# quan-dao/practical-collab-perception

Measured on AMD Instinct MI355X. Metric: frames/sec (60k-pt cloud, 6 agents), higher is better.
Workload: dtype f32

## Files before the change

include/pcp_hip.h:

```cpp
#ifndef PCP_HIP_H
#define PCP_HIP_H

#include <stddef.h>
#include <stdint.h>

#ifdef __cplusplus
extern "C" {
#endif

#define PCP_ABI_VERSION 1

enum {
  PCP_OK = 0,
  PCP_ERR_ARG = 1,
  PCP_ERR_WORKSPACE = 2,
  PCP_ERR_LAUNCH = 3,
  PCP_ERR_UNSUPPORTED = 4
};

int pcp_abi_version(void);
const char *pcp_status_string(int status);

enum {
  PCP_OPT_PFN_CROWD = 0,
  PCP_OPT_PFN_CROWD_BLOCKS = 1,
  PCP_OPT_PFN_WPS = 2,
  PCP_OPT_WINO4C_NW = 3,
  PCP_OPT_MP_TH16_MIN = 4,
  PCP_OPT_MP_DIAG = 5,
  PCP_OPT_VOX_AGGREGATE = 6,
  PCP_OPT_CONV_S2_FORM = 7,
  PCP_OPT_GTS_PASTE_FORM = 8,
  PCP_OPT_COUNT = 9
};
int pcp_set_option(int32_t option, int64_t value);
int64_t pcp_get_option(int32_t option);

typedef struct {
  float min_x, min_y, min_z;
  float voxel_x, voxel_y, voxel_z;
  int32_t nx, ny;
  int32_t batch_size;
} pcp_grid_t;

#define PCP_VOX_COUNTERS 4

size_t pcp_voxelize_workspace_bytes(const pcp_grid_t *grid, int64_t max_points);

int pcp_voxelize(const float *points, int64_t n, int32_t row_stride, const pcp_grid_t *grid,
                 void *workspace, size_t workspace_bytes,
                 int32_t *voxel_coords, int64_t *unq_inv, int32_t *unq_cnt, int32_t *counters, void *stream);
int pcp_voxelize_cells_ready(const float *points, int64_t n, int32_t row_stride, const pcp_grid_t *grid,
                             void *workspace, size_t workspace_bytes,
                             int32_t *voxel_coords, int32_t *unq_cnt, int32_t *counters, void *stream);

int pcp_voxelize_sort_pillar_rows(const pcp_grid_t *grid, void *workspace, int64_t n, void *stream);
int pcp_voxelize_row_order(const pcp_grid_t *grid, const void *workspace, int64_t n, int32_t *order, int32_t *cursor_scratch,
                           void *stream);

int pcp_pfn_scatter(const float *points, int64_t n, int32_t row_stride, int32_t num_raw, const pcp_grid_t *grid,
                    const void *workspace, const float *w0, const float *b0, const float *w1, const float *b1,
                    float *pillar_features, float *canvas, void *stream);

#define PCP_ROWS_CELLS_READY 1
#define PCP_ROWS_BUCKET_ORDER 2
size_t pcp_pillarise_rows_workspace_bytes(const pcp_grid_t *grid, int64_t max_points, int32_t num_raw);
int pcp_pillarise_rows(const float *points, int64_t n, int32_t row_stride, int32_t num_raw, const pcp_grid_t *grid,
                       void *workspace, size_t workspace_bytes, int32_t *voxel_coords, int64_t *unq_inv, int32_t *unq_cnt,
                       int32_t *counters, int32_t flags, void *stream);
int pcp_pfn_rows(const pcp_grid_t *grid, const void *workspace, int64_t n, int32_t num_raw, const float *w0, const float *b0,
                 const float *w1, const float *b1, float *pillar_features, float *canvas, void *stream);
int pcp_pillar_index_export(const pcp_grid_t *grid, const void *workspace, int64_t n, int32_t num_raw, int32_t *voxel_coords,
                            int32_t *row_rank, int32_t *slot_rank, int32_t *slot_canvas_row, int32_t *counters, void *stream);

#define PCP_PFN_ABSOLUTE_XYZ 1u
#define PCP_PFN_WITH_DISTANCE 2u
int pcp_pfn_features(const float *points, int64_t n, int32_t row_stride, int32_t num_raw, uint32_t flags, const pcp_grid_t *grid,
                     const void *vox_workspace, int32_t fw, float *fbuf, int32_t *slot_pillar, void *stream);
int pcp_pfn_cat_pillar_max(const float *y, int32_t ld_y, const float *pillar_max, int32_t ld_max, const int32_t *slot_pillar, int64_t rows,
                           int32_t c, float *out, int32_t ld_out, void *stream);

int pcp_canvas_clear(const pcp_grid_t *grid, const void *workspace, int64_t n, float *canvas, void *stream);
int pcp_fill_zero(void *ptr, size_t bytes, void *stream);

typedef struct {
  int32_t batch, in_h, in_w;
  int32_t cin, cout;
  int32_t cout_pad;
  int32_t stride;
  int32_t ld_in, ld_out;
  int32_t relu;
} pcp_conv3x3_t;

int pcp_conv3x3(const pcp_conv3x3_t *desc, const float *in, const float *w_packed, const float *bias, float *out,
                void *stream);

int pcp_sparse_conv3x3_s2(const float *pillar_features, const pcp_grid_t *grid, const void *vox_workspace, int64_t n,
                          const float *w_packed, const float *bias, int32_t cout, int32_t relu, float *out, int32_t ld_out,
                          void *stream);

int pcp_conv3x3_winograd(const pcp_conv3x3_t *desc, const float *in, const float *u_packed, const float *bias, float *out,
                         void *stream);

int pcp_conv3x3_winograd_ws_supported(const pcp_conv3x3_t *desc);
int pcp_conv3x3_winograd_ws(const pcp_conv3x3_t *desc, const float *in, const float *u_packed, const float *bias, float *out,
                            void *stream);
int pcp_conv3x3_winograd_ws_plan(const pcp_conv3x3_t *desc, int32_t *variant, double *executed_flops);

int pcp_conv3x3_winograd4f(const pcp_conv3x3_t *desc, const float *in, const float *u_packed, const float *bias, float *out,
                           void *stream);
int pcp_conv3x3_winograd4f_plan(const pcp_conv3x3_t *desc, double *executed_flops);

int pcp_conv3x3_winograd4h(const pcp_conv3x3_t *desc, const float *in, const float *u_packed, const float *bias, float *out,
                           void *stream);
int pcp_conv3x3_winograd4h_plan(const pcp_conv3x3_t *desc, double *executed_flops);

int pcp_conv3x3_winograd4c(const pcp_conv3x3_t *desc, const float *in, const float *u_packed, const float *bias, float *out,
                           void *stream);
int pcp_conv3x3_winograd4c_plan(const pcp_conv3x3_t *desc, double *executed_flops);

int pcp_conv3x3_winograd_plan(const pcp_conv3x3_t *desc, int32_t *variant, double *executed_flops);

int pcp_conv3x3_winograd4_workspace_bytes(const pcp_conv3x3_t *desc, size_t *bytes);
int pcp_conv3x3_winograd4(const pcp_conv3x3_t *desc, const float *in, const float *u_packed, const float *bias, float *out,
                          void *workspace, void *stream);
int pcp_conv3x3_winograd4_timed(const pcp_conv3x3_t *desc, const float *in, const float *u_packed, const float *bias, float *out,
                                void *workspace, void *stream, float *stage_ms_host, double *gemm_flops_host);

int pcp_conv3x3_bf16x3(const pcp_conv3x3_t *desc, const float *in, const void *w_packed, const float *bias, float *out, void *stream);
int pcp_conv3x3_bf16(const pcp_conv3x3_t *desc, const float *in, const void *w_packed, const float *bias, float *out, void *stream);

int pcp_conv3x3_grouped_small(const float *in, int32_t batch, int32_t h, int32_t w, int32_t ld_in, int32_t groups,
                              int32_t cin_per_group, const int32_t *group_out_offsets_host, const float *weights, const float *bias, float *out,
                              int32_t ld_out, void *stream);

enum {
  PCP_PW_PLAIN = 0,
  PCP_PW_SPACE2DEPTH = 1,
  PCP_PW_DEPTH2SPACE = 2
};

typedef struct {
  int32_t mode;
  int64_t rows;
  int32_t batch, in_h, in_w;
  int32_t cin, cout, cout_pad;
  int32_t ld_in, ld_out;
  int32_t relu;
  const float *in2;
  int32_t ld_in2, k_split;
  const float *residual;
  int32_t ld_res;
} pcp_pointwise_t;

int pcp_pointwise(const pcp_pointwise_t *desc, const float *in, const float *w_packed, const float *bias, float *out,
                  void *stream);

typedef struct {
  int32_t batch, h, w, ld;
  int32_t num_class;
  int32_t ch_center, ch_z, ch_dim, ch_rot, ch_hm;
  int32_t k;
  float stride;
  float voxel_x, voxel_y, min_x, min_y;
  float limit[6];
  int32_t use_score_thresh;
  float score_thresh;
  int32_t activated;
} pcp_decode_t;

size_t pcp_decode_workspace_bytes(const pcp_decode_t *desc);
int pcp_centerhead_decode(const pcp_decode_t *desc, const float *head, void *workspace, size_t workspace_bytes,
                          float *boxes, float *scores, int32_t *labels, int32_t *cell, int32_t *count, void *stream);

#define PCP_DET_MAX_HEADS 8
typedef struct {
  const float *boxes;
  const float *scores;
  const int32_t *labels;
  const int32_t *keep;
  const int32_t *keep_count;
  const int32_t *class_map;
  int32_t k, keep_max;
} pcp_det_head_t;
int pcp_gather_detections(const pcp_det_head_t *heads, int32_t n_heads, int32_t batch, int32_t out_max, float *out_boxes,
                          float *out_scores, int64_t *out_labels, int32_t *out_count, void *stream);
// ... 129 lines not shown
```

practical-collab-perception_amd/csrc/abi.hip:

```cpp
#include "pcp_common.h"

extern "C" int pcp_abi_version(void) { return PCP_ABI_VERSION; }

extern "C" const char *pcp_status_string(int status) {
  switch (status) {
    case PCP_OK: return "ok";
    case PCP_ERR_ARG: return "bad argument";
    case PCP_ERR_WORKSPACE: return "workspace too small";
    case PCP_ERR_LAUNCH: return "kernel launch failed";
    case PCP_ERR_UNSUPPORTED: return "unsupported shape for this build";
    default: return "unknown status";
  }
}

#include <atomic>

namespace {
std::atomic<long long> g_option[PCP_OPT_COUNT] = {{-1}, {-1}, {-1}, {-1}, {-1}, {-1}, {-1}, {-1}, {-1}};
static_assert(PCP_OPT_COUNT == 9, "one initialiser per option");
constexpr int MAX_DEVICES = 64;
std::atomic<int> g_cus[MAX_DEVICES];
}

extern "C" int pcp_set_option(int32_t option, int64_t value) {
  if (option < 0 || option >= PCP_OPT_COUNT) return PCP_ERR_ARG;
  g_option[option].store(value < 0 ? -1 : (long long)value, std::memory_order_relaxed);
  return PCP_OK;
}

extern "C" int64_t pcp_get_option(int32_t option) {
  if (option < 0 || option >= PCP_OPT_COUNT) return -1;
  return g_option[option].load(std::memory_order_relaxed);
}

long long pcp_option(int option, long long builtin) {
  const long long v = g_option[option].load(std::memory_order_relaxed);
  return v < 0 ? builtin : v;
}

int pcp_current_device_cus() {
  int dev = 0;
  if (hipGetDevice(&dev) != hipSuccess || dev < 0 || dev >= MAX_DEVICES) return 256;
  int v = g_cus[dev].load(std::memory_order_relaxed);
  if (v > 0) return v;
  if (hipDeviceGetAttribute(&v, hipDeviceAttributeMultiprocessorCount, dev) != hipSuccess || v <= 0) v = 256;
  g_cus[dev].store(v, std::memory_order_relaxed);
  return v;
}
```

practical-collab-perception_amd/csrc/wino4c.hip:

```cpp
#include "wino4_common.h"
#include <type_traits>

namespace {

constexpr int H4_LDS_FLOATS = H4_MAIN_FLOATS;
constexpr int H4_VRING = 2;

template <int NW>
__global__ __launch_bounds__(NW * 64, NW == 4 ? 2 : 1) void k_wino4c(H4Params p) {
  constexpr int THREADS = NW * 64;
  constexpr int RAW_PER = (H4_RAW_ITEMS + THREADS - 1) / THREADS;
  constexpr int WBN = NW * 16;
  constexpr int URING = NW == 4 ? H4_URING : 2;
  __shared__ __attribute__((aligned(16))) float lds[H4_LDS_FLOATS];
  float *rawb = lds;
  float *vb = lds + 2 * H4_RAW_FLOATS;

  const int tid = threadIdx.x;
  const int lane = tid & 63;
  const int wave = __builtin_amdgcn_readfirstlane(tid >> 6);
  const int h = lane >> 5;

  const int lid = xcd_remap(blockIdx.x, gridDim.x);
  const int nt = lid / p.n_spatial;
  int sp = lid % p.n_spatial;
  const int tile_x = sp % p.tiles_x;
  sp /= p.tiles_x;
  const int tile_y = sp % p.tiles_y;
  const int b = sp / p.tiles_y;
  const int oy0 = tile_y * 16, ox0 = tile_x * 16;
  const int n0 = nt * WBN;

  const __amdgpu_buffer_rsrc_t in_rsrc = __builtin_amdgcn_make_buffer_rsrc(const_cast<float *>(p.in), 0, p.in_bytes, 0x00020000);
  unsigned roff[RAW_PER];
  int rdst[RAW_PER];
#pragma unroll
  for (int i = 0; i < RAW_PER; i++) {
    int idx = tid + i * THREADS;
    if (idx >= H4_RAW_ITEMS) idx -= H4_RAW_ITEMS;
    const int q = idx & 1, pix = idx >> 1;
    const int py = pix / H4_RAW_W, px = pix % H4_RAW_W;
    const int iy = oy0 - 1 + py, ix = ox0 - 1 + px;
    rdst[i] = (4 * q) * H4_PLANE + py * H4_RP + px;
    roff[i] = 0x80000000u;
    if (iy >= 0 && iy < p.h && ix >= 0 && ix < p.w) roff[i] = (unsigned)((((long long)(b * p.h + iy) * p.w + ix) * p.ld_in + q * 4) * 4);
  }
  f32x4 rreg[RAW_PER];
  auto raw_load = [&](int slice) {
    const int soff = slice * (H4_CK * 4);
#pragma unroll
    for (int i = 0; i < RAW_PER; i++)
      rreg[i] = __builtin_bit_cast(f32x4, __builtin_amdgcn_raw_buffer_load_b128(in_rsrc, (int)roff[i], soff, 0));
  };
  auto raw_store = [&](int buf) {
    float *dst = rawb + buf * H4_RAW_FLOATS;
#pragma unroll
    for (int i = 0; i < RAW_PER; i++) {
      const f32x4 v = rreg[i];
      dst[rdst[i]] = v.x;
      dst[rdst[i] + H4_PLANE] = v.y;
      dst[rdst[i] + 2 * H4_PLANE] = v.z;
      dst[rdst[i] + 3 * H4_PLANE] = v.w;
    }
  };

  const int t_li = lane & 31;
  const bool tf = NW == 4 || wave < 4;
  const int t_tile = t_li & 15, t_ch = 2 * (wave & 3) + (t_li >> 4);
  const int t_src = t_ch * H4_PLANE + (4 * (t_tile >> 2) + 3 * h) * H4_RP + 4 * (t_tile & 3);
  const int t_dst = t_ch * 16 + t_tile + (3 * h) * H4_VP;
  const H4Transform transform{rawb, vb, t_src, t_dst};

  const __amdgpu_buffer_rsrc_t u_rsrc = __builtin_amdgcn_make_buffer_rsrc(const_cast<float *>(p.u), 0, p.u_bytes, 0x00020000);
  const int u_lane = lane * 16;
  const int u_slice = (p.cout_pad / 16) * (18 * 64 * 4 * 4);
  const int u_base = (nt * NW + wave) * (18 * 64 * 4 * 4);
  const int n_slices = p.cin / H4_CK;
  const int last = n_slices - 1;
  f32x4 uq[18];
  auto u_load = [&](int slice, int q) {
    const int so = u_base + min(slice, last) * u_slice + q * (64 * 4 * 4);
    uq[q] = __builtin_bit_cast(f32x4, __builtin_amdgcn_raw_buffer_load_b128(u_rsrc, u_lane, so, 0));
  };

  f32x4 acc[36];
#pragma unroll
  for (int i = 0; i < 36; i++) acc[i] = f32x4{0.f, 0.f, 0.f, 0.f};

  const int v_off = lane;
  float vq[H4_VRING][4][2];
  f32x4 lo[3];
  float2 hi[3];

  auto step_blocks = [&](int s, auto last_tag) {
    constexpr bool LAST = decltype(last_tag)::value;
    const int cur = s & 1, nxt = cur ^ 1;
    const float *vsrc = vb + cur * H4_V_FLOATS + v_off;
    float *tdst = vb + nxt * H4_V_FLOATS + t_dst;
    float *rdstb = rawb + cur * H4_RAW_FLOATS;
    auto mm = [&](int pi) {
      const f32x4 ua = uq[2 * pi], ub = uq[2 * pi + 1];
      float (&v)[4][2] = vq[pi % H4_VRING];
      acc[4 * pi + 0] = __builtin_amdgcn_mfma_f32_16x16x4f32(ua.x, v[0][0], acc[4 * pi + 0], 0, 0, 0);
      acc[4 * pi + 1] = __builtin_amdgcn_mfma_f32_16x16x4f32(ua.z, v[1][0], acc[4 * pi + 1], 0, 0, 0);
      acc[4 * pi + 2] = __builtin_amdgcn_mfma_f32_16x16x4f32(ub.x, v[2][0], acc[4 * pi + 2], 0, 0, 0);
      acc[4 * pi + 3] = __builtin_amdgcn_mfma_f32_16x16x4f32(ub.z, v[3][0], acc[4 * pi + 3], 0, 0, 0);
      acc[4 * pi + 0] = __builtin_amdgcn_mfma_f32_16x16x4f32(ua.y, v[0][1], acc[4 * pi + 0], 0, 0, 0);
      acc[4 * pi + 1] = __builtin_amdgcn_mfma_f32_16x16x4f32(ua.w, v[1][1], acc[4 * pi + 1], 0, 0, 0);
      acc[4 * pi + 2] = __builtin_amdgcn_mfma_f32_16x16x4f32(ub.y, v[2][1], acc[4 * pi + 2], 0, 0, 0);
      acc[4 * pi + 3] = __builtin_amdgcn_mfma_f32_16x16x4f32(ub.w, v[3][1], acc[4 * pi + 3], 0, 0, 0);
      if (pi + H4_VRING < 9) {
#pragma unroll
        for (int j = 0; j < 4; j++) {
          v[j][0] = vsrc[(4 * (pi + H4_VRING) + j) * H4_VP];
          v[j][1] = vsrc[(4 * (pi + H4_VRING) + j) * H4_VP + 64];
        }
      }
#pragma unroll
      for (int e = 0; e < 2; e++) {
        const int q = 2 * (pi + URING) + e;
        if (q < 18) u_load(s, q);
        else if (!LAST) u_load(s + 1, q - 18);
      }
    };
    auto rstore = [&](int i) {
      const f32x4 v = rreg[i];
      rdstb[rdst[i]] = v.x;
      rdstb[rdst[i] + H4_PLANE] = v.y;
      rdstb[rdst[i] + 2 * H4_PLANE] = v.z;
      rdstb[rdst[i] + 3 * H4_PLANE] = v.w;
    };
    const auto fence = [] { __builtin_amdgcn_sched_barrier(0); };
    fence();
    float wr[3][6];
    float top[3][3], bot[3][3];
    auto other = [&](int blk) {
      if (blk == 0) rstore(0);
      if (blk == 1) rstore(1);
      if (blk == 2 && RAW_PER > 2) rstore(RAW_PER > 2 ? 2 : 0);
      if (blk == 3) raw_load(min(s + 3, last));
      if (!tf) return;
      if (blk == 1) bt6(lo[0].x, lo[0].y, lo[0].z, lo[0].w, hi[0].x, hi[0].y, wr[0]);
      if (blk == 2) bt6(lo[1].x, lo[1].y, lo[1].z, lo[1].w, hi[1].x, hi[1].y, wr[1]);
      if (blk == 3) bt6(lo[2].x, lo[2].y, lo[2].z, lo[2].w, hi[2].x, hi[2].y, wr[2]);
      if (blk == 4) {
#pragma unroll
        for (int rr = 0; rr < 3; rr++)
#pragma unroll
          for (int c = 0; c < 3; c++) {
            const auto sw = __builtin_amdgcn_permlane32_swap(__float_as_uint(wr[rr][c]), __float_as_uint(wr[rr][3 + c]), false, false);
            top[rr][c] = __uint_as_float(sw[0]);
            bot[rr][c] = __uint_as_float(sw[1]);
          }
      }
      if (blk >= 5 && blk <= 7) {
        const int c = blk - 5;
        float o[6];
        bt6(top[0][c], top[1][c], top[2][c], bot[0][c], bot[1][c], bot[2][c], o);
#pragma unroll
        for (int i = 0; i < 6; i++) tdst[(i * 6 + c) * H4_VP] = o[i];
      }
    };
#pragma unroll
    for (int blk = 0; blk < 8; blk++) {
      mm(blk);
      fence();
      if (!LAST) {
        other(blk);
        fence();
      }
    }
    if (!LAST) {
      __syncthreads();
      const float *vn = vb + nxt * H4_V_FLOATS + v_off;
      const float *tn = rawb + cur * H4_RAW_FLOATS + t_src;
#pragma unroll
      for (int i = 0; i < H4_VRING; i++)
        if (i != 8 % H4_VRING) {
#pragma unroll
          for (int j = 0; j < 4; j++) {
            vq[i][j][0] = vn[(4 * i + j) * H4_VP];
            vq[i][j][1] = vn[(4 * i + j) * H4_VP + 64];
          }
        }
      if (tf) {
#pragma unroll
        for (int rr = 0; rr < 3; rr++) {
          lo[rr] = *reinterpret_cast<const f32x4 *>(tn + rr * H4_RP);
          hi[rr] = *reinterpret_cast<const float2 *>(tn + rr * H4_RP + 4);
        }
      }
      fence();
      mm(8);
      fence();
#pragma unroll
      for (int j = 0; j < 4; j++) {
        vq[8 % H4_VRING][j][0] = vn[(4 * (8 % H4_VRING) + j) * H4_VP];
        vq[8 % H4_VRING][j][1] = vn[(4 * (8 % H4_VRING) + j) * H4_VP + 64];
      }
      fence();
    } else {
      mm(8);
    }
  };

  {
    f32x4 r0[RAW_PER];
    raw_load(0);
#pragma unroll
    for (int i = 0; i < RAW_PER; i++) r0[i] = rreg[i];
    raw_load(min(1, last));
#pragma unroll
    for (int q = 0; q < 2 * URING; q++) u_load(0, q);
    float *dst = rawb;
#pragma unroll
    for (int i = 0; i < RAW_PER; i++) {
      const f32x4 v = r0[i];
      dst[rdst[i]] = v.x;
      dst[rdst[i] + H4_PLANE] = v.y;
      dst[rdst[i] + 2 * H4_PLANE] = v.z;
      dst[rdst[i] + 3 * H4_PLANE] = v.w;
    }
    if (n_slices > 1) raw_store(1);
    raw_load(min(2, last));
  }
  __syncthreads();
  if (tf) transform(0, 0);
  __syncthreads();
#pragma unroll
  for (int i = 0; i < H4_VRING; i++)
#pragma unroll
    for (int j = 0; j < 4; j++) {
      vq[i][j][0] = vb[v_off + (4 * i + j) * H4_VP];
      vq[i][j][1] = vb[v_off + (4 * i + j) * H4_VP + 64];
    }
  if (tf) {
#pragma unroll
    for (int rr = 0; rr < 3; rr++) {
      lo[rr] = *reinterpret_cast<const f32x4 *>(rawb + H4_RAW_FLOATS + t_src + rr * H4_RP);
      hi[rr] = *reinterpret_cast<const float2 *>(rawb + H4_RAW_FLOATS + t_src + rr * H4_RP + 4);
    }
  }

  for (int s = 0; s < last; s++) step_blocks(s, std::false_type{});
  step_blocks(last, std::true_type{});

  {
    const int e_tile = lane & 15, e_kq = lane >> 4;
    const int n = n0 + 16 * wave + 4 * e_kq;
    if (n < p.cout) {
      const f32x4 bias = *reinterpret_cast<const f32x4 *>(p.bias + n);
      const int py = oy0 + (e_tile >> 2) * 4, px = ox0 + (e_tile & 3) * 4;
      f32x4 t[4][6];
#pragma unroll
      for (int j = 0; j < 6; j++) {
        f32x4 y[4];
        at6v(acc[j], acc[6 + j], acc[12 + j], acc[18 + j], acc[24 + j], acc[30 + j], y);
#pragma unroll
        for (int r = 0; r < 4; r++) t[r][j] = y[r];
      }
#pragma unroll
      for (int r = 0; r < 4; r++) {
        f32x4 y[4];
        at6v(t[r][0], t[r][1], t[r][2], t[r][3], t[r][4], t[r][5], y);
        if (py + r < p.h) {
          float *o = p.out + ((long long)(b * p.h + py + r) * p.w + px) * p.ld_out + n;
#pragma unroll
          for (int c2 = 0; c2 < 4; c2++)
            if (px + c2 < p.w) {
              f32x4 v = y[c2] + bias;
              if (p.relu) {
                v.x = fmaxf(v.x, 0.f);
                v.y = fmaxf(v.y, 0.f);
                v.z = fmaxf(v.z, 0.f);
                v.w = fmaxf(v.w, 0.f);
              }
              __builtin_nontemporal_store(v, reinterpret_cast<f32x4 *>(o + (long long)c2 * p.ld_out));
            }
        }
      }
    }
  }
}

}

extern "C" int pcp_conv3x3_winograd4c(const pcp_conv3x3_t *d, const float *in, const float *u_packed, const float *bias, float *out,
                                      void *stream_) {
  if (!d || !in || !u_packed || !bias || !out) return PCP_ERR_ARG;
  H4Params p;
  int rc = h4_geom(d, &p);
  if (rc != PCP_OK) return rc;
  if ((((uintptr_t)in) & 15) || (((uintptr_t)u_packed) & 15) || (((uintptr_t)out) & 15) || (((uintptr_t)bias) & 15)) return PCP_ERR_ARG;
  p.in = in; p.u = u_packed; p.bias = bias; p.out = out;
  const bool wide = pcp_option(PCP_OPT_WINO4C_NW, 4) == 8 && d->cout_pad % 128 == 0;
  const long long blocks = (long long)p.n_spatial * (d->cout_pad / (wide ? 128 : 64));
  if (blocks <= 0 || blocks > 0x7fffffffLL) return PCP_ERR_ARG;
  if (wide) hipLaunchKernelGGL(k_wino4c<8>, dim3((unsigned)blocks), dim3(512), 0, (hipStream_t)stream_, p);
  else hipLaunchKernelGGL(k_wino4c<4>, dim3((unsigned)blocks), dim3(256), 0, (hipStream_t)stream_, p);
  PCP_CHECK_LAUNCH();
  return PCP_OK;
}

extern "C" int pcp_conv3x3_winograd4c_plan(const pcp_conv3x3_t *d, double *executed_flops) {
  H4Params p;
  int rc = h4_geom(d, &p);
  if (rc != PCP_OK) return rc;
  if (executed_flops) *executed_flops = (double)p.n_spatial * (d->cout_pad / H4_WBN) * 2.0 * 36.0 * 16.0 * d->cin * H4_WBN;
  return PCP_OK;
}
```

practical-collab-perception_amd/pcp_amd/lib.py:

```python
import ctypes
import os

_HERE = os.path.dirname(os.path.abspath(__file__))
LIB_PATH = os.environ.get('PCP_HIP_LIB') or os.path.abspath(os.path.join(_HERE, '..', 'lib', 'libpcp_hip.so'))

c_f = ctypes.c_float
c_i32 = ctypes.c_int32
c_i64 = ctypes.c_int64
c_sz = ctypes.c_size_t
vp = ctypes.c_void_p


class Grid(ctypes.Structure):
    _fields_ = [('min_x', c_f), ('min_y', c_f), ('min_z', c_f), ('voxel_x', c_f), ('voxel_y', c_f), ('voxel_z', c_f),
                ('nx', c_i32), ('ny', c_i32), ('batch_size', c_i32)]


class PackJob(ctypes.Structure):
    _fields_ = [('w', ctypes.c_void_p), ('cout', ctypes.c_int32), ('cin', ctypes.c_int32), ('transpose', ctypes.c_int32),
                ('direct_cout_pad', ctypes.c_int32), ('direct', ctypes.c_void_p), ('winograd', ctypes.c_void_p),
                ('winograd_cout_pad', ctypes.c_int32), ('f4_cout_pad', ctypes.c_int32), ('u4f', ctypes.c_void_p), ('u4h', ctypes.c_void_p),
                ('block_start', ctypes.c_int32), ('reserved', ctypes.c_int32)]


# ... 213 lines not shown
                                             ctypes.POINTER(ctypes.c_uint8), vp, c_i64, vp, c_sz, vp, ctypes.POINTER(Grid), vp, c_sz, vp]),
    'pcp_select_transform_compact_dev': (c_i32, [vp, c_i64, c_i32, c_i32, c_i32, ctypes.POINTER(c_f), c_i32, vp, vp, vp, c_i64, vp, c_sz, vp,
                                                 ctypes.POINTER(Grid), vp, c_sz, vp]),
    'pcp_warp_nearest_batch_dev': (c_i32, [vp, vp, vp, c_i32, c_i32, c_i32, c_i32, c_i32, c_i32, c_i32, vp]),
    'pcp_voxelize_cells_ready': (c_i32, [vp, c_i64, c_i32, ctypes.POINTER(Grid), vp, c_sz, vp, vp, vp, vp]),
    'pcp_gather_detections': (c_i32, [ctypes.POINTER(DetHead), c_i32, c_i32, c_i32, vp, vp, vp, vp, vp]),
    'pcp_nms_workspace_bytes': (c_sz, [c_i32, c_i32]),
    'pcp_nms_rotated': (c_i32, [vp, vp, c_i32, c_i32, vp, c_f, c_i32, c_i32, vp, c_sz, vp, vp, vp]),
    'pcp_nms_normal': (c_i32, [vp, vp, c_i32, c_i32, vp, c_f, c_i32, c_i32, vp, c_sz, vp, vp, vp]),
    'pcp_boxes_bev_pairwise': (c_i32, [vp, c_i32, vp, c_i32, c_i32, vp, vp]),
    'pcp_warp_nearest': (c_i32, [vp, vp, c_i32, c_i32, c_i32, c_i32, c_i32, ctypes.POINTER(c_f), c_i32, vp]),
    'pcp_warp_nearest_batch': (c_i32, [vp, vp, ctypes.POINTER(c_f), c_i32, c_i32, c_i32, c_i32, c_i32, c_i32, c_i32, vp]),
    'pcp_softmax_fuse': (c_i32, [ctypes.POINTER(vp), c_i32, vp, c_i32, c_i64, c_i32, c_i32, c_i32, vp, vp]),
    'pcp_disco_weight_fuse': (c_i32, [ctypes.POINTER(vp), c_i32, c_i32, c_i32, c_i64, vp, vp, vp, vp, vp, vp, vp, c_i32, vp, c_i32, vp]),
    'pcp_disco_weight_fuse_live': (c_i32, [ctypes.POINTER(vp), c_i32, c_i32, c_i32, c_i64, vp, vp, vp, vp, vp, vp, vp, c_i32, ctypes.POINTER(c_i32), vp, vp]),
    'pcp_bev_sample_bilinear': (c_i32, [vp, c_i32, c_i32, c_i32, c_i32, c_i32, vp, c_i64, c_i32, c_f, c_f, c_f, c_f, vp, vp,
                                        c_i32, vp]),
    'pcp_hunter_point_head': (c_i32, [vp, c_i32, c_i32, c_i32, c_i32, c_i32, vp, c_i64, c_i32, c_f, c_f, c_f, c_f, vp, vp, vp, vp, vp,
                                      vp, c_i32, c_i32, vp, c_i32, vp, vp]),
    'pcp_hunter_point_head_ex': (c_i32, [vp, c_i32, c_i32, c_i32, c_i32, c_i32, vp, c_i64, c_i32, c_f, c_f, c_f, c_f, vp, vp, vp, vp, vp,
                                         vp, c_i32, c_i32, vp, c_i32, vp, vp, vp, c_i32, c_f, vp, vp]),
    'pcp_voxelize_row_order': (c_i32, [ctypes.POINTER(Grid), vp, c_i64, vp, vp, vp]),
    'pcp_voxelize_sort_pillar_rows': (c_i32, [ctypes.POINTER(Grid), vp, c_i64, vp]),
    'pcp_hunter_apply_flow': (c_i32, [vp, c_i64, c_i32, vp, c_i32, c_f, vp, vp]),
    'pcp_select_transform_points': (c_i32, [vp, c_i64, c_i32, c_i32, c_f, c_i32, ctypes.POINTER(c_f), ctypes.POINTER(ctypes.c_uint8),
                                            vp, c_i32, vp]),
    'pcp_bev_scatter_mean_workspace_bytes': (c_sz, [c_i32, c_i32, c_i32, c_i64]),
    'pcp_bev_scatter_mean': (c_i32, [vp, c_i64, c_i32, vp, c_i32, c_i32, c_i32, c_i32, c_i32, c_f, c_f, c_f, c_f, vp, c_sz,
                                     vp, c_i32, vp]),
    'pcp_anchor_decode': (c_i32, [ctypes.POINTER(Anchor), vp, vp, vp, vp, vp, vp, vp]),
    'pcp_topk_boxes': (c_i32, [vp, vp, vp, c_i32, c_i64, c_i32, vp, vp, vp, vp, vp, vp]),
    'pcp_points_in_boxes': (c_i32, [vp, c_i32, c_i32, c_i32, vp, c_i32, c_i32, vp, vp]),
    'pcp_hunter_foreground_workspace_bytes': (c_sz, [c_i64]),
    'pcp_hunter_foreground_rows': (c_i32, [vp, c_i64, c_i32, vp, c_i32, c_f, vp, c_sz, vp, vp, vp, vp]),
    'pcp_modar_ingest_batched_workspace_bytes': (c_sz, [c_i32, c_i64]),
    'pcp_modar_ingest_batched': (c_i32, [vp, vp, vp, vp, c_i32, c_i32, vp, c_i32, vp, vp, c_i64, vp, vp, vp, vp, c_sz, vp, vp]),
    'pcp_modar_ingest': (c_i32, [vp, c_i32, vp, c_i32, c_i32, ctypes.POINTER(ctypes.c_double), c_f, vp, vp]),
}

SYMBOLS.update({
    'pcp_bn_workspace_bytes': (c_sz, [c_i32]),
    'pcp_bn_train_stats': (c_i32, [vp, c_i64, c_i32, c_i32, vp, vp, c_f, c_f, vp, vp, vp, vp, vp, vp, vp, vp]),
    'pcp_scale_shift_act': (c_i32, [vp, c_i64, c_i32, c_i32, vp, vp, c_i32, vp, c_i32, vp]),
    'pcp_bn_act_backward': (c_i32, [vp, c_i32, vp, c_i32, c_i64, c_i32, vp, vp, vp, vp, c_i32, vp, vp, vp, c_i32, vp, c_i32, vp]),
    'pcp_colsum': (c_i32, [vp, c_i64, c_i32, c_i32, vp, vp, c_i32, vp]),
    'pcp_bn_train_sums': (c_i32, [vp, c_i64, c_i32, c_i32, vp, vp, vp]),
    'pcp_bn_train_stats_from_sums': (c_i32, [vp, c_i64, c_i32, vp, vp, c_f, c_f, vp, vp, vp, vp, vp, vp, vp]),
    'pcp_bn_bwd_sums': (c_i32, [vp, c_i32, vp, c_i32, c_i64, c_i32, vp, vp, vp, vp, c_i32, vp, vp, vp]),
    'pcp_bn_bwd_apply_from_sums': (c_i32, [vp, c_i32, vp, c_i32, c_i64, c_i32, vp, vp, vp, vp, c_i32, vp, vp, c_i64, vp, vp, vp, c_i32, vp, c_i32, vp]),
    'pcp_accumulate': (c_i32, [vp, c_i32, vp, c_i32, c_i64, c_i32, c_f, vp]),
    'pcp_dilate2x': (c_i32, [vp, c_i32, c_i32, c_i32, c_i32, c_i32, vp, c_i32, vp]),
    'pcp_conv3x3_wgrad_workspace_bytes': (c_sz, [ctypes.POINTER(Conv3x3)]),
    'pcp_conv3x3_wgrad': (c_i32, [ctypes.POINTER(Conv3x3), vp, vp, vp, c_sz, vp, c_i32, vp]),
    'pcp_pointwise_wgrad_workspace_bytes': (c_sz, [c_i64, c_i32, c_i32]),
    'pcp_pointwise_wgrad': (c_i32, [ctypes.POINTER(RowMap), ctypes.POINTER(RowMap), c_i64, vp, c_sz, vp, c_i32, c_i32, vp]),
    'pcp_centerhead_targets': (c_i32, [ctypes.POINTER(Target), vp, c_i32, vp, vp, vp, vp, vp]),
    'pcp_loss_workspace_bytes': (c_sz, []),
    'pcp_centerhead_loss': (c_i32, [ctypes.POINTER(HeadLoss), vp, vp, vp, vp, vp, c_f, vp, vp, vp, vp]),
    'pcp_centerhead_targets_ext': (c_i32, [ctypes.POINTER(Target), ctypes.POINTER(TargetHead), c_i32, vp, c_i32, c_i32, c_i32, vp]),
    'pcp_centerhead_loss_ext_workspace_bytes': (c_sz, [c_i32]),
    'pcp_centerhead_loss_ext': (c_i32, [ctypes.POINTER(HeadLossExt), ctypes.POINTER(HeadLossHead), c_i32, c_f, vp, c_sz, vp, vp, vp]),
    'pcp_anchor_assign_workspace_bytes': (c_sz, [ctypes.POINTER(AnchorAssign), c_i32]),
    'pcp_anchor_assign_targets': (c_i32, [ctypes.POINTER(AnchorAssign), vp, vp, c_i32, vp, c_sz, vp, vp, vp, vp]),
    'pcp_anchor_loss_workspace_bytes': (c_sz, [c_i32]),
    'pcp_anchor_loss': (c_i32, [ctypes.POINTER(AnchorLoss), vp, vp, vp, vp, c_f, vp, c_sz, vp, vp, vp]),
    'pcp_hunter_meta_workspace_bytes': (c_sz, [ctypes.POINTER(HunterMeta), c_i64]),
    'pcp_hunter_meta': (c_i32, [ctypes.POINTER(HunterMeta), vp, c_i64, c_i32, vp, c_sz, vp, vp, vp, vp, vp, vp, vp, vp, vp]),
    'pcp_segment_max': (c_i32, [vp, c_i32, vp, c_i64, vp, c_i64, c_i32, vp, c_i32, vp, vp]),
    'pcp_segment_max_backward': (c_i32, [vp, c_i32, vp, c_i64, c_i32, vp, vp, c_i32, vp]),
    'pcp_rows_scatter_add': (c_i32, [vp, c_i32, vp, c_i64, c_i32, vp, c_i32, vp]),
    'pcp_hunter_local_centroids': (c_i32, [vp, c_i32, vp, vp, c_i32, c_i32, vp, c_sz, vp, vp, c_i32, vp]),
    'pcp_hunter_object_cat': (c_i32, [vp, vp, vp, vp, vp, c_i32, c_i32, vp, c_i32, vp]),
    'pcp_hunter_object_cat_backward': (c_i32, [vp, c_i32, vp, vp, c_i32, c_i32, c_i32, vp, vp, vp]),
    'pcp_hunter_loss_workspace_bytes': (c_sz, [c_i64, c_i32, c_i32, c_i32]),
    'pcp_hunter_losses': (c_i32, [ctypes.POINTER(HunterLoss), vp, c_sz, vp]),
    'pcp_softmax_fuse2_backward': (c_i32, [vp, c_i32, vp, c_i32, vp, c_i32, c_i64, c_i32, vp, c_i32, vp, c_i32, vp]),
    'pcp_bev_scatter_mean_backward': (c_i32, [vp, c_i32, c_i32, c_i32, c_i64, vp, c_i32, c_i32, vp, vp, c_i32, vp, c_i32, vp]),
    'pcp_bev_sample_bilinear_backward': (c_i32, [vp, c_i32, vp, vp, c_i64, c_i32, vp, c_i32, c_i32, c_i32, c_i32, c_i32, c_f, c_f, c_f, c_f, vp,
                                                 c_i32, vp, c_i32, vp]),
    'pcp_filter_gt_boxes': (c_i32, [vp, c_i32, c_i32, ctypes.POINTER(c_f), vp, vp]),
    'pcp_filter_gt_boxes_w': (c_i32, [vp, c_i32, c_i32, c_i32, ctypes.POINTER(c_f), vp, vp]),
    'pcp_distill_loss': (c_i32, [vp, c_i32, vp, c_i32, c_i64, c_i32, c_f, c_f, vp, vp, vp, c_i32, c_i32, vp]),
    'pcp_masked_smooth_l1_rows': (c_i32, [vp, c_i32, vp, c_i32, c_i64, c_i32, c_f, vp, vp, vp]),
    'pcp_pfn_train_features': (c_i32, [vp, c_i64, c_i32, c_i32, ctypes.POINTER(Grid), vp, vp, vp, vp]),
    'pcp_pfn_train_features_w': (c_i32, [vp, c_i64, c_i32, c_i32, c_i32, ctypes.POINTER(Grid), vp, vp, vp, vp]),
    'pcp_pfn_train_mid': (c_i32, [ctypes.POINTER(Grid), vp, c_i64, vp, vp, vp, vp, vp, vp]),
    'pcp_pfn_train_out': (c_i32, [ctypes.POINTER(Grid), vp, c_i64, vp, vp, vp, vp, vp, vp, vp]),
    'pcp_pfn_train_route_out_grad': (c_i32, [ctypes.POINTER(Grid), vp, c_i64, c_i64, vp, vp, vp, vp, vp]),
    'pcp_pfn_train_route_mid_grad': (c_i32, [ctypes.POINTER(Grid), vp, c_i64, vp, vp, vp, vp]),
    'pcp_disco_weight_logits': (c_i32, [ctypes.POINTER(vp), c_i32, c_i32, vp, vp, c_i64, vp, c_i32, vp]),
    'pcp_disco_fuse_backward_workspace_bytes': (c_sz, []),
    'pcp_disco_fuse_backward': (c_i32, [ctypes.POINTER(vp), c_i32, c_i32, c_i32, vp, c_i32, vp, c_i32, ctypes.POINTER(vp), c_i32, vp,
                                        c_i64, vp, c_i32, ctypes.POINTER(vp), vp, vp, vp, c_i32, vp]),
    'pcp_grad_sqnorm': (c_i32, [vp, c_i64, vp, c_i32, vp]),
    'pcp_pack_conv3x3': (c_i32, [vp, c_i32, c_i32, c_i32, vp, c_i32, vp, c_i32, vp, c_i32, vp]),
    'pcp_pack_conv3x3_winograd4': (c_i32, [vp, c_i32, c_i32, c_i32, vp, vp, c_i32, vp]),
    'pcp_pack_conv3x3_group_blocks': (c_i32, [vp]),
    'pcp_pack_conv3x3_group': (c_i32, [vp, c_i32, c_i32, vp]),
    'pcp_adam_step': (c_i32, [vp, vp, vp, vp, c_i64, c_f, c_f, c_f, c_f, c_f, c_i64, c_f, vp, c_f, vp]),
    'pcp_avgpool_nhwc_backward': (c_i32, [vp, c_i32, c_i32, c_i32, c_i32, c_i32, c_i32, vp, c_i32, c_i32, vp]),
    'pcp_sc_gate_backward': (c_i32, [vp, c_i32, vp, c_i32, vp, c_i32, vp, c_i32, c_i32, c_i32, vp, c_i32, vp, c_i32, vp, c_i32, c_i32, vp, c_i32,
                                     c_i32, c_i32, c_i32, c_i32, vp]),
    'pcp_add_relu': (c_i32, [vp, c_i32, vp, c_i32, vp, c_i32, c_i64, c_i32, vp]),
    'pcp_add_relu_backward': (c_i32, [vp, c_i32, vp, c_i32, vp, c_i32, vp, c_i32, c_i64, c_i32, vp]),
    'pcp_world_augment_points_workspace_bytes': (c_sz, [c_i64]),
    'pcp_world_augment_points': (c_i32, [ctypes.POINTER(WorldAug), vp, vp, c_i64, c_i32, vp, vp, vp, c_sz, vp]),
    'pcp_world_augment_boxes': (c_i32, [ctypes.POINTER(WorldAug), vp, vp, c_i32, c_i32, vp, c_i32, c_i32, vp]),
    'pcp_object_augment_boxes': (c_i32, [ctypes.POINTER(ObjectAug), vp, vp, c_i32, c_i32, vp, vp, vp]),
    'pcp_object_augment_points_workspace_bytes': (c_sz, [c_i64]),
    'pcp_object_augment_points': (c_i32, [ctypes.POINTER(ObjectAug), vp, vp, c_i32, vp, vp, c_i64, c_i32, vp, vp, vp, c_sz, vp]),
    'pcp_frame_extent_workspace_bytes': (c_sz, [c_i64, c_i32]),
    'pcp_frame_extent': (c_i32, [vp, c_i64, c_i32, c_i32, c_i32, vp, vp, c_sz, vp]),
    'pcp_object_augment_drop_boxes': (c_i32, [vp, c_i32, c_i32, c_i32, vp, c_i32, c_i32, vp, vp, c_i32, vp, vp, vp, vp, vp]),
    'pcp_gt_sample_select': (c_i32, [vp, c_i32, c_i32, c_i32, vp, c_i32, vp, vp, c_i32, vp, c_i32, vp, c_i32, vp, vp]),
    'pcp_gt_sample_paste_points': (c_i32, [vp, c_i64, c_i32, c_i32, vp, c_i32, vp, c_i32, vp, vp, vp, vp, c_i32, c_i64, vp, vp, vp]),
    'pcp_gt_sample_paste_boxes': (c_i32, [vp, c_i32, c_i32, c_i32, vp, c_i32, c_i32, vp, c_i32, vp, c_i32, vp, vp, vp, vp, vp, c_i32, vp]),
})

SYMBOLS.update({
    'pcp_mp_bn_train_stats': (c_i32, [vp, c_i32, c_i64, c_i32, c_i32, vp, vp, c_f, c_f, vp, vp, vp, vp, vp, vp, vp, vp]),
    'pcp_mp_scale_shift_act': (c_i32, [vp, c_i32, c_i64, c_i32, c_i32, vp, vp, c_i32, vp, c_i32, c_i32, vp]),
    'pcp_mp_bn_act_backward': (c_i32, [vp, c_i32, c_i32, vp, c_i32, c_i32, c_i64, c_i32, vp, vp, vp, vp, c_i32, vp, vp, vp, c_i32, vp, c_i32,
                                       c_i32, vp]),
    'pcp_mp_bn_train_sums': (c_i32, [vp, c_i32, c_i64, c_i32, c_i32, vp, vp, vp]),
    'pcp_mp_bn_bwd_sums': (c_i32, [vp, c_i32, c_i32, vp, c_i32, c_i32, c_i64, c_i32, vp, vp, vp, vp, c_i32, vp, vp, vp]),
    'pcp_mp_bn_bwd_apply_from_sums': (c_i32, [vp, c_i32, c_i32, vp, c_i32, c_i32, c_i64, c_i32, vp, vp, vp, vp, c_i32, vp, vp, c_i64, vp, vp, vp,
                                              c_i32, vp, c_i32, c_i32, vp]),
    'pcp_mp_colsum': (c_i32, [vp, c_i32, c_i64, c_i32, c_i32, vp, vp, c_i32, vp]),
    'pcp_mp_accumulate': (c_i32, [vp, c_i32, c_i32, vp, c_i32, c_i32, c_i64, c_i32, c_f, vp]),
    'pcp_mp_dilate2x': (c_i32, [vp, c_i32, c_i32, c_i32, c_i32, c_i32, c_i32, vp, c_i32, vp]),
    'pcp_mp_pfn_train_mid': (c_i32, [ctypes.POINTER(Grid), vp, c_i64, vp, vp, vp, vp, c_i32, vp, vp]),
    'pcp_mp_pfn_train_out': (c_i32, [ctypes.POINTER(Grid), vp, c_i64, vp, c_i32, vp, vp, vp, vp, vp, c_i32, vp]),
    'pcp_mp_pfn_train_route_out_grad': (c_i32, [ctypes.POINTER(Grid), vp, c_i64, c_i64, vp, c_i32, vp, vp, vp, c_i32, vp]),
    'pcp_mp_pfn_train_route_mid_grad': (c_i32, [ctypes.POINTER(Grid), vp, c_i64, vp, c_i32, vp, vp, vp]),
    'pcp_mp_sparse_conv3x3_s2': (c_i32, [vp, ctypes.POINTER(Grid), vp, c_i64, vp, vp, c_i32, c_i32, vp, c_i32, c_i32, vp]),
    'pcp_mp_conv3x3_packed_bytes': (c_sz, [c_i32, c_i32]),
    'pcp_mp_pack_conv3x3': (c_i32, [vp, c_i32, c_i32, c_i32, vp, vp, c_i32, vp]),
    'pcp_mp_pack_conv3x3_group_blocks': (c_i32, [vp]),
    'pcp_mp_pack_conv3x3_group': (c_i32, [vp, c_i32, c_i32, vp]),
    'pcp_mp_conv3x3': (c_i32, [ctypes.POINTER(MpConv3x3), vp, vp, vp, vp, vp]),
    'pcp_mp_conv3x3_plan': (c_i32, [ctypes.POINTER(MpConv3x3), ctypes.POINTER(c_i32), ctypes.POINTER(ctypes.c_double)]),
    'pcp_mp_conv3x3_wgrad_workspace_bytes': (c_sz, [ctypes.POINTER(MpWgrad3x3)]),
    'pcp_mp_conv3x3_wgrad': (c_i32, [ctypes.POINTER(MpWgrad3x3), vp, vp, vp, vp, c_sz, vp]),
    'pcp_mp_pointwise': (c_i32, [ctypes.POINTER(MpPointwise), vp, vp, vp, vp, vp]),
    'pcp_mp_warp_nearest': (c_i32, [vp, c_i32, vp, c_i32, c_i32, c_i32, c_i32, c_i32, c_i32, ctypes.POINTER(c_f), c_i32, vp]),
    'pcp_mp_softmax_fuse': (c_i32, [ctypes.POINTER(vp), c_i32, c_i32, vp, c_i32, c_i64, c_i32, c_i32, c_i32, vp, vp]),
    'pcp_mp_disco_fuse_backward': (c_i32, [ctypes.POINTER(vp), c_i32, c_i32, c_i32, c_i32, vp, c_i32, vp, c_i32, ctypes.POINTER(vp), c_i32, vp, c_i64,
                                           vp, c_i32, ctypes.POINTER(vp), vp, vp, vp, c_i32, vp]),
    'pcp_mp_pointwise_wgrad_workspace_bytes': (c_sz, [c_i64, c_i32, c_i32]),
    'pcp_mp_pointwise_wgrad': (c_i32, [ctypes.POINTER(MpRowMap), ctypes.POINTER(MpRowMap), c_i64, vp, c_sz, vp, c_i32, c_i32, vp]),
})

OPTIONS = {'pfn_crowd': 0, 'pfn_crowd_blocks': 1, 'pfn_wps': 2, 'wino4c_nw': 3, 'mp_th16_min': 4, 'mp_diag': 5, 'vox_aggregate': 6,
           'conv_s2_form': 7, 'gts_paste_form': 8}
_OPTION_ENV = {'PCP_PFN_CROWD': 'pfn_crowd', 'PCP_PFN_CROWD_BLOCKS': 'pfn_crowd_blocks', 'PCP_PFN_WPS': 'pfn_wps', 'PCP_WINO4C_NW': 'wino4c_nw',
               'PCP_MP_TH16_MIN': 'mp_th16_min', 'PCP_MP_DIAG': 'mp_diag', 'PCP_VOX_AGGREGATE': 'vox_aggregate', 'PCP_CONV_S2_FORM': 'conv_s2_form', 'PCP_GTS_PASTE_FORM': 'gts_paste_form'}

_LIB = None


class PcpError(RuntimeError):
    pass


def load():
    global _LIB
    if _LIB is not None:
        return _LIB
    if not os.path.isfile(LIB_PATH):
        raise PcpError('libpcp_hip.so not found at %s -- build it with `make -C practical-collab-perception_amd/csrc` '
                       '(or python -c "import __graft_entry__ as g; g.build()"); there is no CPU fallback.' % LIB_PATH)
    import torch
    lib = ctypes.CDLL(LIB_PATH)
    for name, (res, args) in SYMBOLS.items():
        fn = getattr(lib, name)
        fn.restype = res
        fn.argtypes = args
    if lib.pcp_abi_version() != 1:
        raise PcpError('libpcp_hip.so ABI version mismatch')
    for env, name in _OPTION_ENV.items():
        v = os.environ.get(env, '')
        if v.strip():
            if lib.pcp_set_option(OPTIONS[name], int(v)) != 0:
                raise PcpError('%s=%s: pcp_set_option refused it' % (env, v))
    _LIB = lib
    return lib


def set_option(name, value):
    lib = load()
    prev = int(lib.pcp_get_option(OPTIONS[name]))
    check(lib.pcp_set_option(OPTIONS[name], -1 if value is None else int(value)), 'pcp_set_option')
    return None if prev < 0 else prev


def check(status, what):
    if status != 0:
        raise PcpError('%s failed: %s' % (what, load().pcp_status_string(status).decode()))
```

Before: 403.6.

## Pack Winograd V tiles in LDS for 128-bit reads in wino4c

Adds a second LDS layout for the transformed input tiles in the wino4c Winograd conv kernel. The transform writes four channels per slot contiguously, so the MFMA loop can fetch each block's V operands with two 16-byte LDS reads. Before, each block took eight scalar reads. The paired layout is the default through a new option, and the old layout stays selectable. In exchange, the LDS footprint and the store pattern change, which may add bank conflicts on the write side or lower occupancy.

```diff
diff --git a/include/pcp_hip.h b/include/pcp_hip.h
--- a/include/pcp_hip.h
+++ b/include/pcp_hip.h
@@ -31,7 +31,8 @@
   PCP_OPT_VOX_AGGREGATE = 6,
   PCP_OPT_CONV_S2_FORM = 7,
   PCP_OPT_GTS_PASTE_FORM = 8,
-  PCP_OPT_COUNT = 9
+  PCP_OPT_WINO4C_VFORM = 9,
+  PCP_OPT_COUNT = 10
 };
 int pcp_set_option(int32_t option, int64_t value);
 int64_t pcp_get_option(int32_t option);
diff --git a/practical-collab-perception_amd/csrc/abi.hip b/practical-collab-perception_amd/csrc/abi.hip
--- a/practical-collab-perception_amd/csrc/abi.hip
+++ b/practical-collab-perception_amd/csrc/abi.hip
@@ -16,8 +16,8 @@
 #include <atomic>
 
 namespace {
-std::atomic<long long> g_option[PCP_OPT_COUNT] = {{-1}, {-1}, {-1}, {-1}, {-1}, {-1}, {-1}, {-1}, {-1}};
-static_assert(PCP_OPT_COUNT == 9, "one initialiser per option");
+std::atomic<long long> g_option[PCP_OPT_COUNT] = {{-1}, {-1}, {-1}, {-1}, {-1}, {-1}, {-1}, {-1}, {-1}, {-1}};
+static_assert(PCP_OPT_COUNT == 10, "one initialiser per option");
 constexpr int MAX_DEVICES = 64;
 std::atomic<int> g_cus[MAX_DEVICES];
 }
diff --git a/practical-collab-perception_amd/csrc/wino4c.hip b/practical-collab-perception_amd/csrc/wino4c.hip
--- a/practical-collab-perception_amd/csrc/wino4c.hip
+++ b/practical-collab-perception_amd/csrc/wino4c.hip
@@ -6,13 +6,52 @@
 constexpr int H4_LDS_FLOATS = H4_MAIN_FLOATS;
 constexpr int H4_VRING = 2;
 
-template <int NW>
+constexpr int H4_VFORM_RULE = 2;
+constexpr int H4_VQP = 256;
+constexpr int H4_VQ_FLOATS = 18 * H4_VQP;
+constexpr int H4_LDS2_FLOATS = 2 * H4_RAW_FLOATS + 2 * H4_VQ_FLOATS;
+__device__ constexpr int h4_vq_off(int i, int c) { return 3 * i * H4_VQP + (c == 2 ? H4_VQP : 0); }
+
+struct H4TransformQ {
+  float *rawb, *vb;
+  int t_src, t_dst, t_dst1;
+  __device__ void operator()(int rbuf, int vbuf) const {
+    const float *src = rawb + rbuf * H4_RAW_FLOATS + t_src;
+    float *dst = vb + vbuf * H4_VQ_FLOATS;
+    float wr[3][6];
+#pragma unroll
+    for (int rr = 0; rr < 3; rr++) {
+      const f32x4 lo = *reinterpret_cast<const f32x4 *>(src + rr * H4_RP);
+      const float2 hi = *reinterpret_cast<const float2 *>(src + rr * H4_RP + 4);
+      bt6(lo.x, lo.y, lo.z, lo.w, hi.x, hi.y, wr[rr]);
+    }
+    float top[3][3], bot[3][3];
+#pragma unroll
+    for (int rr = 0; rr < 3; rr++)
+#pragma unroll
+      for (int c = 0; c < 3; c++) {
+        const auto sw = __builtin_amdgcn_permlane32_swap(__float_as_uint(wr[rr][c]), __float_as_uint(wr[rr][3 + c]), false, false);
+        top[rr][c] = __uint_as_float(sw[0]);
+        bot[rr][c] = __uint_as_float(sw[1]);
+      }
+#pragma unroll
+    for (int c = 0; c < 3; c++) {
+      float o[6];
+      bt6(top[0][c], top[1][c], top[2][c], bot[0][c], bot[1][c], bot[2][c], o);
+#pragma unroll
+      for (int i = 0; i < 6; i++) dst[(c == 1 ? t_dst1 : t_dst) + h4_vq_off(i, c)] = o[i];
+    }
+  }
+};
+
+template <int NW, int VF>
 __global__ __launch_bounds__(NW * 64, NW == 4 ? 2 : 1) void k_wino4c(H4Params p) {
   constexpr int THREADS = NW * 64;
   constexpr int RAW_PER = (H4_RAW_ITEMS + THREADS - 1) / THREADS;
   constexpr int WBN = NW * 16;
   constexpr int URING = NW == 4 ? H4_URING : 2;
-  __shared__ __attribute__((aligned(16))) float lds[H4_LDS_FLOATS];
+  constexpr int VFL = VF == 1 ? H4_V_FLOATS : H4_VQ_FLOATS;
+  __shared__ __attribute__((aligned(16))) float lds[VF == 1 ? H4_LDS_FLOATS : H4_LDS2_FLOATS];
   float *rawb = lds;
   float *vb = lds + 2 * H4_RAW_FLOATS;
 
@@ -66,10 +105,15 @@
 
   const int t_li = lane & 31;
   const bool tf = NW == 4 || wave < 4;
-  const int t_tile = t_li & 15, t_ch = 2 * (wave & 3) + (t_li >> 4);
+  const int t_tile = t_li & 15, t_ch = VF == 1 ? 2 * (wave & 3) + (t_li >> 4) : (wave & 3) + 4 * (t_li >> 4);
   const int t_src = t_ch * H4_PLANE + (4 * (t_tile >> 2) + 3 * h) * H4_RP + 4 * (t_tile & 3);
-  const int t_dst = t_ch * 16 + t_tile + (3 * h) * H4_VP;
-  const H4Transform transform{rawb, vb, t_src, t_dst};
+  const int t_slot = 4 * ((t_ch & 3) * 16 + t_tile) + (t_ch >> 2);
+  const int t_dst = VF == 1 ? t_ch * 16 + t_tile + (3 * h) * H4_VP : t_slot + h * (H4_VQP + 2);
+  const int t_dst1 = t_slot + 2 + h * (2 * H4_VQP - 2);
+  const auto transform = [&] {
+    if constexpr (VF == 1) return H4Transform{rawb, vb, t_src, t_dst};
+    else return H4TransformQ{rawb, vb, t_src, t_dst, t_dst1};
+  }();
 
   const __amdgpu_buffer_rsrc_t u_rsrc = __builtin_amdgcn_make_buffer_rsrc(const_cast<float *>(p.u), 0, p.u_bytes, 0x00020000);
   const int u_lane = lane * 16;
@@ -87,35 +131,55 @@
 #pragma unroll
   for (int i = 0; i < 36; i++) acc[i] = f32x4{0.f, 0.f, 0.f, 0.f};
 
-  const int v_off = lane;
+  const int v_off = VF == 1 ? lane : 4 * lane;
   float vq[H4_VRING][4][2];
+  f32x4 vp[H4_VRING][2];
+  auto v_fill = [&](int slot, const float *src, int blk) {
+    if constexpr (VF == 1) {
+#pragma unroll
+      for (int j = 0; j < 4; j++) {
+        vq[slot][j][0] = src[(4 * blk + j) * H4_VP];
+        vq[slot][j][1] = src[(4 * blk + j) * H4_VP + 64];
+      }
+    } else {
+#pragma unroll
+      for (int e = 0; e < 2; e++) vp[slot][e] = *reinterpret_cast<const f32x4 *>(src + (2 * blk + e) * H4_VQP);
+    }
+  };
   f32x4 lo[3];
   float2 hi[3];
 
   auto step_blocks = [&](int s, auto last_tag) {
     constexpr bool LAST = decltype(last_tag)::value;
     const int cur = s & 1, nxt = cur ^ 1;
-    const float *vsrc = vb + cur * H4_V_FLOATS + v_off;
-    float *tdst = vb + nxt * H4_V_FLOATS + t_dst;
+    const float *vsrc = vb + cur * VFL + v_off;
+    float *tdst = vb + nxt * VFL + t_dst;
+    float *tdst1 = vb + nxt * VFL + t_dst1;
     float *rdstb = rawb + cur * H4_RAW_FLOATS;
     auto mm = [&](int pi) {
       const f32x4 ua = uq[2 * pi], ub = uq[2 * pi + 1];
-      float (&v)[4][2] = vq[pi % H4_VRING];
-      acc[4 * pi + 0] = __builtin_amdgcn_mfma_f32_16x16x4f32(ua.x, v[0][0], acc[4 * pi + 0], 0, 0, 0);
-      acc[4 * pi + 1] = __builtin_amdgcn_mfma_f32_16x16x4f32(ua.z, v[1][0], acc[4 * pi + 1], 0, 0, 0);
-      acc[4 * pi + 2] = __builtin_amdgcn_mfma_f32_16x16x4f32(ub.x, v[2][0], acc[4 * pi + 2], 0, 0, 0);
-      acc[4 * pi + 3] = __builtin_amdgcn_mfma_f32_16x16x4f32(ub.z, v[3][0], acc[4 * pi + 3], 0, 0, 0);
-      acc[4 * pi + 0] = __builtin_amdgcn_mfma_f32_16x16x4f32(ua.y, v[0][1], acc[4 * pi + 0], 0, 0, 0);
-      acc[4 * pi + 1] = __builtin_amdgcn_mfma_f32_16x16x4f32(ua.w, v[1][1], acc[4 * pi + 1], 0, 0, 0);
-      acc[4 * pi + 2] = __builtin_amdgcn_mfma_f32_16x16x4f32(ub.y, v[2][1], acc[4 * pi + 2], 0, 0, 0);
-      acc[4 * pi + 3] = __builtin_amdgcn_mfma_f32_16x16x4f32(ub.w, v[3][1], acc[4 * pi + 3], 0, 0, 0);
-      if (pi + H4_VRING < 9) {
-#pragma unroll
-        for (int j = 0; j < 4; j++) {
-          v[j][0] = vsrc[(4 * (pi + H4_VRING) + j) * H4_VP];
-          v[j][1] = vsrc[(4 * (pi + H4_VRING) + j) * H4_VP + 64];
-        }
-      }
+      if constexpr (VF == 1) {
+        float (&v)[4][2] = vq[pi % H4_VRING];
+        acc[4 * pi + 0] = __builtin_amdgcn_mfma_f32_16x16x4f32(ua.x, v[0][0], acc[4 * pi + 0], 0, 0, 0);
+        acc[4 * pi + 1] = __builtin_amdgcn_mfma_f32_16x16x4f32(ua.z, v[1][0], acc[4 * pi + 1], 0, 0, 0);
+        acc[4 * pi + 2] = __builtin_amdgcn_mfma_f32_16x16x4f32(ub.x, v[2][0], acc[4 * pi + 2], 0, 0, 0);
+        acc[4 * pi + 3] = __builtin_amdgcn_mfma_f32_16x16x4f32(ub.z, v[3][0], acc[4 * pi + 3], 0, 0, 0);
+        acc[4 * pi + 0] = __builtin_amdgcn_mfma_f32_16x16x4f32(ua.y, v[0][1], acc[4 * pi + 0], 0, 0, 0);
+        acc[4 * pi + 1] = __builtin_amdgcn_mfma_f32_16x16x4f32(ua.w, v[1][1], acc[4 * pi + 1], 0, 0, 0);
+        acc[4 * pi + 2] = __builtin_amdgcn_mfma_f32_16x16x4f32(ub.y, v[2][1], acc[4 * pi + 2], 0, 0, 0);
+        acc[4 * pi + 3] = __builtin_amdgcn_mfma_f32_16x16x4f32(ub.w, v[3][1], acc[4 * pi + 3], 0, 0, 0);
+      } else {
+        const f32x4 va = vp[pi % H4_VRING][0], vc = vp[pi % H4_VRING][1];
+        acc[4 * pi + 0] = __builtin_amdgcn_mfma_f32_16x16x4f32(ua.x, va.x, acc[4 * pi + 0], 0, 0, 0);
+        acc[4 * pi + 1] = __builtin_amdgcn_mfma_f32_16x16x4f32(ua.z, va.z, acc[4 * pi + 1], 0, 0, 0);
+        acc[4 * pi + 2] = __builtin_amdgcn_mfma_f32_16x16x4f32(ub.x, vc.x, acc[4 * pi + 2], 0, 0, 0);
+        acc[4 * pi + 3] = __builtin_amdgcn_mfma_f32_16x16x4f32(ub.z, vc.z, acc[4 * pi + 3], 0, 0, 0);
+        acc[4 * pi + 0] = __builtin_amdgcn_mfma_f32_16x16x4f32(ua.y, va.y, acc[4 * pi + 0], 0, 0, 0);
+        acc[4 * pi + 1] = __builtin_amdgcn_mfma_f32_16x16x4f32(ua.w, va.w, acc[4 * pi + 1], 0, 0, 0);
+        acc[4 * pi + 2] = __builtin_amdgcn_mfma_f32_16x16x4f32(ub.y, vc.y, acc[4 * pi + 2], 0, 0, 0);
+        acc[4 * pi + 3] = __builtin_amdgcn_mfma_f32_16x16x4f32(ub.w, vc.w, acc[4 * pi + 3], 0, 0, 0);
+      }
+      if (pi + H4_VRING < 9) v_fill(pi % H4_VRING, vsrc, pi + H4_VRING);
 #pragma unroll
       for (int e = 0; e < 2; e++) {
         const int q = 2 * (pi + URING) + e;
@@ -158,7 +222,10 @@
         float o[6];
         bt6(top[0][c], top[1][c], top[2][c], bot[0][c], bot[1][c], bot[2][c], o);
 #pragma unroll
-        for (int i = 0; i < 6; i++) tdst[(i * 6 + c) * H4_VP] = o[i];
+        for (int i = 0; i < 6; i++) {
+          if constexpr (VF == 1) tdst[(i * 6 + c) * H4_VP] = o[i];
+          else (c == 1 ? tdst1 : tdst)[h4_vq_off(i, c)] = o[i];
+        }
       }
     };
 #pragma unroll
@@ -172,17 +239,11 @@
     }
     if (!LAST) {
       __syncthreads();
-      const float *vn = vb + nxt * H4_V_FLOATS + v_off;
+      const float *vn = vb + nxt * VFL + v_off;
       const float *tn = rawb + cur * H4_RAW_FLOATS + t_src;
 #pragma unroll
       for (int i = 0; i < H4_VRING; i++)
-        if (i != 8 % H4_VRING) {
-#pragma unroll
-          for (int j = 0; j < 4; j++) {
-            vq[i][j][0] = vn[(4 * i + j) * H4_VP];
-            vq[i][j][1] = vn[(4 * i + j) * H4_VP + 64];
-          }
-        }
+        if (i != 8 % H4_VRING) v_fill(i, vn, i);
       if (tf) {
 #pragma unroll
         for (int rr = 0; rr < 3; rr++) {
@@ -193,11 +254,7 @@
       fence();
       mm(8);
       fence();
-#pragma unroll
-      for (int j = 0; j < 4; j++) {
-        vq[8 % H4_VRING][j][0] = vn[(4 * (8 % H4_VRING) + j) * H4_VP];
-        vq[8 % H4_VRING][j][1] = vn[(4 * (8 % H4_VRING) + j) * H4_VP + 64];
-      }
+      v_fill(8 % H4_VRING, vn, 8 % H4_VRING);
       fence();
     } else {
       mm(8);
@@ -228,12 +285,7 @@
   if (tf) transform(0, 0);
   __syncthreads();
 #pragma unroll
-  for (int i = 0; i < H4_VRING; i++)
-#pragma unroll
-    for (int j = 0; j < 4; j++) {
-      vq[i][j][0] = vb[v_off + (4 * i + j) * H4_VP];
-      vq[i][j][1] = vb[v_off + (4 * i + j) * H4_VP + 64];
-    }
+  for (int i = 0; i < H4_VRING; i++) v_fill(i, vb + v_off, i);
   if (tf) {
 #pragma unroll
     for (int rr = 0; rr < 3; rr++) {
@@ -294,10 +346,17 @@
   if ((((uintptr_t)in) & 15) || (((uintptr_t)u_packed) & 15) || (((uintptr_t)out) & 15) || (((uintptr_t)bias) & 15)) return PCP_ERR_ARG;
   p.in = in; p.u = u_packed; p.bias = bias; p.out = out;
   const bool wide = pcp_option(PCP_OPT_WINO4C_NW, 4) == 8 && d->cout_pad % 128 == 0;
+  const long long vform = pcp_option(PCP_OPT_WINO4C_VFORM, 0);
+  if (vform != 0 && vform != 1 && vform != 2) return PCP_ERR_ARG;
+  const bool paired = (vform == 0 ? H4_VFORM_RULE : vform) == 2;
   const long long blocks = (long long)p.n_spatial * (d->cout_pad / (wide ? 128 : 64));
   if (blocks <= 0 || blocks > 0x7fffffffLL) return PCP_ERR_ARG;
-  if (wide) hipLaunchKernelGGL(k_wino4c<8>, dim3((unsigned)blocks), dim3(512), 0, (hipStream_t)stream_, p);
-  else hipLaunchKernelGGL(k_wino4c<4>, dim3((unsigned)blocks), dim3(256), 0, (hipStream_t)stream_, p);
+  const dim3 grid((unsigned)blocks);
+  hipStream_t st = (hipStream_t)stream_;
+  if (wide && paired) hipLaunchKernelGGL((k_wino4c<8, 2>), grid, dim3(512), 0, st, p);
+  else if (wide) hipLaunchKernelGGL((k_wino4c<8, 1>), grid, dim3(512), 0, st, p);
+  else if (paired) hipLaunchKernelGGL((k_wino4c<4, 2>), grid, dim3(256), 0, st, p);
+  else hipLaunchKernelGGL((k_wino4c<4, 1>), grid, dim3(256), 0, st, p);
   PCP_CHECK_LAUNCH();
   return PCP_OK;
 }
diff --git a/practical-collab-perception_amd/pcp_amd/lib.py b/practical-collab-perception_amd/pcp_amd/lib.py
--- a/practical-collab-perception_amd/pcp_amd/lib.py
+++ b/practical-collab-perception_amd/pcp_amd/lib.py
@@ -389,9 +389,10 @@
 })
 
 OPTIONS = {'pfn_crowd': 0, 'pfn_crowd_blocks': 1, 'pfn_wps': 2, 'wino4c_nw': 3, 'mp_th16_min': 4, 'mp_diag': 5, 'vox_aggregate': 6,
-           'conv_s2_form': 7, 'gts_paste_form': 8}
+           'conv_s2_form': 7, 'gts_paste_form': 8, 'wino4c_vform': 9}
 _OPTION_ENV = {'PCP_PFN_CROWD': 'pfn_crowd', 'PCP_PFN_CROWD_BLOCKS': 'pfn_crowd_blocks', 'PCP_PFN_WPS': 'pfn_wps', 'PCP_WINO4C_NW': 'wino4c_nw',
-               'PCP_MP_TH16_MIN': 'mp_th16_min', 'PCP_MP_DIAG': 'mp_diag', 'PCP_VOX_AGGREGATE': 'vox_aggregate', 'PCP_CONV_S2_FORM': 'conv_s2_form', 'PCP_GTS_PASTE_FORM': 'gts_paste_form'}
+               'PCP_MP_TH16_MIN': 'mp_th16_min', 'PCP_MP_DIAG': 'mp_diag', 'PCP_VOX_AGGREGATE': 'vox_aggregate', 'PCP_CONV_S2_FORM': 'conv_s2_form', 'PCP_GTS_PASTE_FORM': 'gts_paste_form',
+               'PCP_WINO4C_VFORM': 'wino4c_vform'}
 
 _LIB = None
 
```

After: 406.6 (median of 6 runs). Within noise of the previous version (+0.8%).
